# tky823/audio_source_separation

Hardware: AMD Instinct MI355X
Metric: ILRMA iterations/sec (4ch, F=1025, T=4096) (higher is better)
Workload: dtype f64; 1 GPU; gauss_ilrma_ip update_once, M=4 F=1025 T=4096 K=4, normalize=power, loss off; utterances_per_gpu=1, power_statistic=covariance, parallelism=utterance-sharded x1, no data-path collective

## Files before the change

audio_source_separation_amd/csrc/assx_bss.hip:

```cpp
#include "assx_common.hpp"
#include "assx_small_linalg.hpp"
#include "assx_stream.hpp"
#include "assx_group_linalg.hpp"
#include "assx_partition.hpp"
#include "assx_cov_wide.hpp"
#include "assx_cov_mfma.hpp"
#include "assx_nmf_internal.hpp"
#include "assx_widem.hpp"

using namespace assx;

namespace {

constexpr int REDUCE_THREADS = 256;

template <typename R, int M>
__device__ __forceinline__ void load_filter(const Cx<R>* __restrict__ W, size_t bf, Cx<R> (&w)[M][M]) {
  const Cx<R>* p = W + bf * (M * M);
#pragma unroll
  for (int n = 0; n < M; ++n)
#pragma unroll
    for (int m = 0; m < M; ++m) w[n][m] = p[n * M + m];
}

// ... 953 lines not shown
      hipLaunchKernelGGL((ip_par_kernel<R, M, false>), gp, bp, 0, st, (const Cx<R>*)U, (const R*)nullptr, fp, 1.0,
                         (Cx<R>*)W, (const Cx<R>*)C, pw, thr, status, B, F, den_floor, 1);
    ASSX_LAUNCH_CHECK(ctx, "ip_par_kernel");
    return 0;
  }
#endif
  const dim3 grid(blocks_for((size_t)B * F, GPW)), block(64);
  if (part)
    hipLaunchKernelGGL((ip_group_kernel<R, M, true>), grid, block, 0, st, (const Cx<R>*)nullptr, (const R*)part, fp,
                       1.0 / (double)T, (Cx<R>*)W, (const Cx<R>*)C, pw, thr, status, B, F, den_floor, wb);
  else
    hipLaunchKernelGGL((ip_group_kernel<R, M, false>), grid, block, 0, st, (const Cx<R>*)U, (const R*)nullptr, fp, 1.0,
                       (Cx<R>*)W, (const Cx<R>*)C, pw, thr, status, B, F, den_floor, 1);
  ASSX_LAUNCH_CHECK(ctx, "ip_group_kernel");
  return 0;
}

template <typename R, int M>
int run_iss(assx_ctx* ctx, const void* U, const void* part, FlatPart fp, int T, void* W, const void* C, double* pw,
            int B, int F, hipStream_t st) {
  constexpr int GPW = WAVE / next_pow2_c(M * M);
  const dim3 grid(blocks_for((size_t)B * F, GPW)), block(64);
  if (part)
    hipLaunchKernelGGL((iss_group_kernel<R, M, true>), grid, block, 0, st, (const Cx<R>*)nullptr, (const R*)part, fp,
                       1.0 / (double)T, (double)T, (Cx<R>*)W, (const Cx<R>*)C, pw, B, F);
  else
    hipLaunchKernelGGL((iss_group_kernel<R, M, false>), grid, block, 0, st, (const Cx<R>*)U, (const R*)nullptr, fp, 1.0,
                       (double)T, (Cx<R>*)W, (const Cx<R>*)C, pw, B, F);
  ASSX_LAUNCH_CHECK(ctx, "iss_group_kernel");
  return 0;
}

template <typename R, int M>
int run_ip2(assx_ctx* ctx, const void* U, const void* part, FlatPart fp, int T, void* W, const void* C, double* pw,
            double thr, int32_t* status, int B, int F, int pm, int pn, hipStream_t st) {
  constexpr int GPW = WAVE / next_pow2_c(M * M);
  const dim3 grid(blocks_for((size_t)B * F, GPW)), block(64);
  if (part)
    hipLaunchKernelGGL((ip2_group_kernel<R, M, true>), grid, block, 0, st, (const Cx<R>*)nullptr, (const R*)part, fp,
                       1.0 / (double)T, (Cx<R>*)W, (const Cx<R>*)C, pw, thr, status, B, F, pm, pn);
  else
    hipLaunchKernelGGL((ip2_group_kernel<R, M, false>), grid, block, 0, st, (const Cx<R>*)U, (const R*)nullptr, fp, 1.0,
                       (Cx<R>*)W, (const Cx<R>*)C, pw, thr, status, B, F, pm, pn);
  ASSX_LAUNCH_CHECK(ctx, "ip2_group_kernel");
  return 0;
}

template <typename R, int MM>
int run_basis_partial(assx_ctx* ctx, const void* X, const void* W, const void* Tb, const void* V, double domain,
                      double eps, void* ws, int B, int F, int T, int K, hipStream_t st, FlatPart* fp_out,
                      double nu = -1.0 ,
                      double* lpart = nullptr , int lstride = 0) {
  NmfArgs<R> a;
  a.nu = (R)nu;
  a.d = Dims{B, F, T, K};
  a.eps = (R)eps;
  a.p1 = make_pow((domain + 2.0) / domain);
  a.fp = flat_basis(B, F, T);
  *fp_out = a.fp;
  const bool d2 = a.p1.mode == POW_SQUARE, k4 = K <= KU;
  const dim3 gb(stream_grid(ctx, a.fp, B)), bb(64);
#define BASIS_LAUNCH(K4V, D2V, DXV, DWV, MW) \
  hipLaunchKernelGGL((basis_stream_kernel<R, MM, K4V, D2V, DXV, DWV, MW>), gb, bb, 0, st, (const Cx<R>*)X, \
                     (const Cx<R>*)W, (const R*)Tb, (const R*)V, (R*)ws, a)
  constexpr size_t vlds = (size_t)VDMA_SLOTS * VTileDma<R, MM * KU>::TILE_BYTES;
#define BASIS_VD(D2V, MW, TDV) \
  hipLaunchKernelGGL((basis_stream_vd_kernel<R, MM, D2V, 2, MW, TDV>), gb, bb, vlds, st, (const Cx<R>*)X, \
                     (const Cx<R>*)W, (const R*)Tb, (const R*)V, (R*)ws, a, (double*)nullptr, 0)
#if ASSX_LAB
  static const int vdma = lab_int("ASSX_BASIS_VDMA", 1);
  if (k4 && !vdma) {
    if (nu >= 0.0) hipLaunchKernelGGL((basis_stream_kernel<R, MM, true, true, 3, 1, 1, true>), gb, bb, 0, st, (const Cx<R>*)X,
                                      (const Cx<R>*)W, (const R*)Tb, (const R*)V, (R*)ws, a);
    else if (d2) BASIS_LAUNCH(true, true, 3, 1, 2);
    else BASIS_LAUNCH(true, false, 2, 1, 1);
  } else
#endif
  if (nu >= 0.0) {
    if (k4) BASIS_VD(true, 2, true);
    else hipLaunchKernelGGL((basis_stream_kernel<R, MM, false, true, 3, 1, 1, true>), gb, bb, 0, st, (const Cx<R>*)X,
                            (const Cx<R>*)W, (const R*)Tb, (const R*)V, (R*)ws, a);
  } else if (k4) {
    if (d2 && lpart)
      hipLaunchKernelGGL((basis_stream_vd_kernel<R, MM, true, 2, 2, false, true>), gb, bb, vlds, st, (const Cx<R>*)X,
                         (const Cx<R>*)W, (const R*)Tb, (const R*)V, (R*)ws, a, lpart, lstride);
    else if (d2) BASIS_VD(true, 2, false);
    else BASIS_VD(false, 1, false);
  } else if (d2) BASIS_LAUNCH(false, true, 3, 1, 1);
  else BASIS_LAUNCH(false, false, 2, 1, 1);
#undef BASIS_VD
#undef BASIS_LAUNCH
  ASSX_LAUNCH_CHECK(ctx, "basis_stream_kernel");
  return 0;
}

template <typename R, int MM>
int run_act_partial(assx_ctx* ctx, const void* X, const void* W, const void* Tb, const void* V, double domain,
                    double eps, void* ws, int B, int F, int T, int K, hipStream_t st, FlatPart* fp_out,
                    double nu = -1.0) {
  NmfArgs<R> a;
  a.nu = (R)nu;
  a.d = Dims{B, F, T, K};
  a.eps = (R)eps;
  a.p1 = make_pow((domain + 2.0) / domain);
  a.fp = flat_act(B, F, T);
  *fp_out = a.fp;
  const bool d2 = a.p1.mode == POW_SQUARE, k4 = K <= KU;
  const dim3 ga(stream_grid(ctx, a.fp, B)), ba(64 * ACT_NH);
#define ACT_LAUNCH(K4V, D2V, DXV, MW) \
  hipLaunchKernelGGL((act_stream_kernel<R, MM, K4V, D2V, DXV, MW>), ga, ba, 0, st, (const Cx<R>*)X, (const Cx<R>*)W, \
                     (const R*)Tb, (const R*)V, (R*)ws, a)
#define ACT_VD(D2V, DXV, MW, TDV) \
  hipLaunchKernelGGL((act_stream_vd_kernel<R, MM, D2V, DXV, MW, TDV>), ga, ba, 0, st, (const Cx<R>*)X, (const Cx<R>*)W, \
                     (const R*)Tb, (const R*)V, (R*)ws, a)
#if ASSX_LAB
  static const int vdma = lab_int("ASSX_ACT_VDMA", 1);
  if (k4 && !vdma) {
    if (nu >= 0.0) hipLaunchKernelGGL((act_stream_kernel<R, MM, true, true, 3, 1, true>), ga, ba, 0, st, (const Cx<R>*)X,
                                      (const Cx<R>*)W, (const R*)Tb, (const R*)V, (R*)ws, a);
    else if (d2) ACT_LAUNCH(true, true, (sizeof(R) == 8 ? 3 : 4), 2);
    else ACT_LAUNCH(true, false, 2, 1);
  } else
#endif
  if (nu >= 0.0) {
    if (k4) ACT_VD(true, 3, 2, true);
    else hipLaunchKernelGGL((act_stream_kernel<R, MM, false, true, 4, 1, true>), ga, ba, 0, st, (const Cx<R>*)X,
                            (const Cx<R>*)W, (const R*)Tb, (const R*)V, (R*)ws, a);
  } else if (k4) {
    if (d2) ACT_VD(true, 3, 2, false);
    else ACT_VD(false, 2, 1, false);
  } else if (d2) ACT_LAUNCH(false, true, 4, 1);
  else ACT_LAUNCH(false, false, 2, 1);
#undef ACT_VD
#undef ACT_LAUNCH
  ASSX_LAUNCH_CHECK(ctx, "act_stream_kernel");
  return 0;
}

template <typename R, int MM>
int run_cov_partial_tv(assx_ctx* ctx, const void* X, const void* Tb, const void* V, int K, double domain, double eps,
                       void* ws, void* U_dense, int B, int F, int T, int dtype, hipStream_t st, FlatPart* fp_out,
                       bool* dense, int* records_wb = nullptr ) {
  static const bool wide = lab_int("ASSX_WIDE_K", 1) != 0;
  static const bool fused = lab_int("ASSX_COV_WIDE", 1) != 0;
  *dense = false;
  if (records_wb) *records_wb = 1;
  if (K <= KU || !wide) return run_cov_partial<R, MM>(ctx, WK_TV, X, nullptr, Tb, V, K, domain, eps, ws, B, F, T, st, fp_out);
  const WsLayout L = ws_layout(B, MM, F, T, K, dtype);
  const PowSpec p2d = make_pow(2.0 / domain);
  static const bool mfma = lab_int("ASSX_COV_MFMA", 1) != 0;
  if (fused && mfma && U_dense && K <= 16 && (size_t)B * MM * K * T * sizeof(R) < 0xffffffffull) {
    const FlatPart fw = flat_cov_wide(B, F, T, 1);
    const Dims d{B, F, T, K};
    const int ks = (K + 3) / 4;
    const size_t ldsm = CovMfmaGeom<R>::lds_bytes(MM, ks);
    unsigned long long* covm_trace = COVM_TRACE ? (unsigned long long*)((char*)ws + L.total - 65536) : nullptr;
#define COVM_LAUNCH(D2V, KSV)                                                                                          \
  do {                                                                                                                 \
    if (ldsm > 64 * 1024) {                                                                                            \
      hipError_t e = hipFuncSetAttribute(reinterpret_cast<const void*>(cov_mfma_kernel<R, MM, D2V, KSV>),              \
                                         hipFuncAttributeMaxDynamicSharedMemorySize, (int)ldsm);                       \
      if (e != hipSuccess) return hip_fail(ctx, e, "hipFuncSetAttribute(cov_mfma_kernel)");                            \
    }                                                                                                                  \
    hipLaunchKernelGGL((cov_mfma_kernel<R, MM, D2V, KSV>), dim3(fw.G), dim3(WAVE * COVW_BINS), ldsm, st,               \
                       (const Cx<R>*)X, (const R*)Tb, (const R*)V, (R*)ws, d, fw, (R)eps, p2d, covm_trace);            \
  } while (0)
    if (p2d.mode == POW_ID) {
      if (ks == 2) COVM_LAUNCH(true, 2);
      else if (ks == 3) COVM_LAUNCH(true, 3);
      else COVM_LAUNCH(true, 4);
    } else {
      if (ks == 2) COVM_LAUNCH(false, 2);
      else if (ks == 3) COVM_LAUNCH(false, 3);
      else COVM_LAUNCH(false, 4);
    }
#undef COVM_LAUNCH
    ASSX_LAUNCH_CHECK(ctx, "cov_mfma_kernel");
    *fp_out = fw;
    if (records_wb) {
      *records_wb = COVW_BINS;
      return 0;
    }
    hipLaunchKernelGGL((cov_wide_finalize_kernel<R, MM>), dim3(blocks_for((size_t)B * MM * F * MM * MM, 256)), dim3(256),
                       0, st, (const R*)ws, (Cx<R>*)U_dense, B, F, fw, (R)(1.0 / (double)T));
    ASSX_LAUNCH_CHECK(ctx, "cov_wide_finalize_kernel");
    *dense = true;
    return 0;
  }
  const int sb = cov_wide_sb<R>(MM * K);
  const size_t lds = sb == 2 ? CovWideGeom<R, 2>::lds_bytes(MM * K) : CovWideGeom<R, 1>::lds_bytes(MM * K);
  if (fused && U_dense && lds <= 144 * 1024 && (size_t)B * MM * K * T * sizeof(R) < 0xffffffffull) {
    const FlatPart fw = flat_cov_wide(B, F, T, sb);
    const Dims d{B, F, T, K};
#define COVW_LAUNCH(D2V, SBV)                                                                                        \
  do {                                                                                                               \
    if (lds > 64 * 1024) {                                                                                           \
      hipError_t e = hipFuncSetAttribute(reinterpret_cast<const void*>(cov_wide_kernel<R, MM, D2V, SBV>),            \
                                         hipFuncAttributeMaxDynamicSharedMemorySize, (int)lds);                      \
      if (e != hipSuccess) return hip_fail(ctx, e, "hipFuncSetAttribute(cov_wide_kernel)");                          \
    }                                                                                                                \
    hipLaunchKernelGGL((cov_wide_kernel<R, MM, D2V, SBV>), dim3(fw.G), dim3(WAVE * COVW_BINS), lds, st,              \
                       (const Cx<R>*)X, (const R*)Tb, (const R*)V, (R*)ws, d, fw, (R)eps, p2d);                      \
  } while (0)
#if ASSX_LAB
    if (sb == 2) {
      if (p2d.mode == POW_ID) COVW_LAUNCH(true, 2);
      else COVW_LAUNCH(false, 2);
    } else
#endif
    if (p2d.mode == POW_ID) COVW_LAUNCH(true, 1);
    else COVW_LAUNCH(false, 1);
#undef COVW_LAUNCH
    ASSX_LAUNCH_CHECK(ctx, "cov_wide_kernel");
    if (records_wb) {
      *records_wb = COVW_BINS;
      *fp_out = fw;
      return 0;
    }
    hipLaunchKernelGGL((cov_wide_finalize_kernel<R, MM>), dim3(blocks_for((size_t)B * MM * F * MM * MM, 256)), dim3(256),
                       0, st, (const R*)ws, (Cx<R>*)U_dense, B, F, fw, (R)(1.0 / (double)T));
    ASSX_LAUNCH_CHECK(ctx, "cov_wide_finalize_kernel");
    *fp_out = fw;
    *dense = true;
    return 0;
  }
  R* rv = (R*)((char*)ws + L.map);
  const dim3 grid(blocks_for(T, 256), blocks_for(F, WIDE_FB), B * MM);
  if (p2d.mode == POW_ID)
    hipLaunchKernelGGL((source_variance_map_kernel<R, true>), grid, dim3(256), 0, st, (const R*)Tb, (const R*)V, rv, F, T,
                       K, p2d);
  else
    hipLaunchKernelGGL((source_variance_map_kernel<R, false>), grid, dim3(256), 0, st, (const R*)Tb, (const R*)V, rv, F,
                       T, K, p2d);
  ASSX_LAUNCH_CHECK(ctx, "source_variance_map_kernel");
  return run_cov_partial<R, MM>(ctx, WK_NFT, X, rv, nullptr, nullptr, 1, 2.0, eps, ws, B, F, T, st, fp_out);
}

}

extern "C" {

int assx_launch_order(int B, int F, int T, int reverse, int* ranges, int capacity) {
  if (B < 1 || F < 1 || T < 1) return ASSX_E_ARG;
  FlatPart fp = flat_cov(B, F, T, 1);
  const int grid = (int)set_launch_order(fp, B, reverse);
  if (ranges) {
    if (capacity < grid) return ASSX_E_ARG;
    for (int bid = 0; bid < grid; ++bid) ranges[bid] = workgroup_range(bid, grid, fp);
  }
  return grid;
}

size_t assx_workspace_bytes(int B, int M, int F, int T, int K, int dtype) {
  if (B < 1 || M < 1 || F < 1 || T < 1) return 0;
  if (widem::handles(M)) return widem::workspace_bytes(B, M, F, T, K, dtype);
  return ws_layout(B, M, F, T, K, dtype).total;
}

int assx_demix(assx_ctx* ctx, const void* X, const void* W, const void* scale, void* Y, int B, int M, int F, int T,
               int dtype, void* stream) {
  CHECK_COMMON(ctx, B, M, F, T);
  ASSX_REQUIRE(ctx, X && W && Y, ASSX_E_NULL, "assx_demix: NULL array");
  if (widem::handles(M)) return widem::demix(ctx, X, W, scale, Y, B, M, F, T, dtype, (hipStream_t)stream);
  hipStream_t st = (hipStream_t)stream;
  return dispatch_rm(ctx, dtype, M, [&](auto rt, auto mt) -> int {
    using R = decltype(rt);
    constexpr int MM = decltype(mt)::value;
    dim3 grid(blocks_for(T, 256), F, B);
    hipLaunchKernelGGL((demix_kernel<R, MM>), grid, dim3(256), 0, st, (const Cx<R>*)X, (const Cx<R>*)W,
                       (const Cx<R>*)scale, (Cx<R>*)Y, Dims{B, F, T, 0});
    ASSX_LAUNCH_CHECK(ctx, "demix_kernel");
    return 0;
  });
}

int assx_ilrma_power_map(assx_ctx* ctx, const void* X, const void* W, void* P, int B, int M, int F, int T, int dtype,
                         void* stream) {
  CHECK_COMMON(ctx, B, M, F, T);
  ASSX_REQUIRE(ctx, X && W && P, ASSX_E_NULL, "assx_ilrma_power_map: NULL array");
  hipStream_t st = (hipStream_t)stream;
  if (widem::handles(M)) return widem::power_map(ctx, X, W, P, B, M, F, T, dtype, st);
  return dispatch_rm(ctx, dtype, M, [&](auto rt, auto mt) -> int {
    using R = decltype(rt);
    constexpr int MM = decltype(mt)::value;
    hipLaunchKernelGGL((demix_power_map_kernel<R, MM>), dim3(blocks_for(T, 256), F, B), dim3(256), 0, st,
                       (const Cx<R>*)X, (const Cx<R>*)W, (R*)P, Dims{B, F, T, 0});
    ASSX_LAUNCH_CHECK(ctx, "demix_power_map_kernel");
    return 0;
  });
}

int assx_cov_accumulate(assx_ctx* ctx, const void* X, const void* r, int r_kind, double eps, void* U, void* ws, int B,
                        int M, int N, int F, int T, int dtype, void* stream) {
  CHECK_COMMON(ctx, B, M, F, T);
  ASSX_REQUIRE(ctx, X && U && ws, ASSX_E_NULL, "assx_cov_accumulate: NULL array");
  ASSX_REQUIRE(ctx, r_kind == ASSX_W_NONE || r_kind == ASSX_W_NT || r_kind == ASSX_W_NFT, ASSX_E_ARG,
               "assx_cov_accumulate: bad r_kind %d", r_kind);
  ASSX_REQUIRE(ctx, r_kind == ASSX_W_NONE ? (N == 1) : (N == M && r != nullptr), ASSX_E_ARG,
               "assx_cov_accumulate: N must be 1 (unweighted) or M with weights, got N=%d M=%d", N, M);
  if (widem::handles(M)) return widem::cov_accumulate(ctx, X, r, r_kind, eps, U, ws, B, M, N, F, T, dtype, (hipStream_t)stream);
  hipStream_t st = (hipStream_t)stream;
  return dispatch_rm(ctx, dtype, M, [&](auto rt, auto mt) -> int {
    using R = decltype(rt);
    constexpr int MM = decltype(mt)::value;
    return run_cov<R, MM>(ctx, r_kind, X, r, nullptr, nullptr, 1, 2.0, eps, U, ws, B, F, T, st);
  });
}

int assx_ip_update(assx_ctx* ctx, const void* U, void* W, double threshold, int32_t* status, int B, int M, int F,
                   int dtype, void* stream) {
  CHECK_COMMON(ctx, B, M, F, 1);
  ASSX_REQUIRE(ctx, U && W, ASSX_E_NULL, "assx_ip_update: NULL array");
  if (widem::handles(M)) return widem::ip_update(ctx, U, W, threshold, status, B, M, F, dtype, (hipStream_t)stream);
  hipStream_t st = (hipStream_t)stream;
  return dispatch_rm(ctx, dtype, M, [&](auto rt, auto mt) -> int {
    using R = decltype(rt);
    constexpr int MM = decltype(mt)::value;
    return run_ip<R, MM>(ctx, U, nullptr, FlatPart{}, 1, W, nullptr, nullptr, threshold, status, B, F, st);
  });
}

int assx_ip2_update(assx_ctx* ctx, const void* U, void* W, double threshold, int32_t* status, int pair_m, int pair_n,
                    int B, int M, int F, int dtype, void* stream) {
  CHECK_COMMON(ctx, B, M, F, 1);
  ASSX_REQUIRE(ctx, U && W, ASSX_E_NULL, "assx_ip2_update: NULL array");
  ASSX_REQUIRE(ctx, pair_m >= 0 && pair_m < M && pair_n >= 0 && pair_n < M && pair_m != pair_n, ASSX_E_ARG,
               "bad update pair (%d, %d) for %d sources", pair_m, pair_n, M);
// ... 831 lines not shown
```

audio_source_separation_amd/csrc/assx_cov_mfma.hpp:

```cpp
#pragma once
#include "assx_cov_wide.hpp"
#include "assx_nmf_mfma.hpp"

#ifndef COVM_TRACE
#define COVM_TRACE 0
#endif
#ifndef COVM_SKIP
#define COVM_SKIP 0
#endif

#if (COVM_SKIP || COVM_TRACE) && !defined(ASSX_PROBE_BUILD)
#error "COVM_SKIP / COVM_TRACE are timing experiments (wrong results by construction): build them with -DASSX_PROBE_BUILD into a probe library, never into libassx.so"
#endif

namespace assx {

template <typename R>
struct CovMfmaRows;
template <>
struct CovMfmaRows<double> {
  static __device__ __forceinline__ int bin_of_row(int i) { return i < COVW_BINS ? i : -1; }
  static __device__ __forceinline__ int bin_of_reg(int lane, int r) { return (lane >> 4) + 4 * r; }
};
template <>
struct CovMfmaRows<float> {
  static __device__ __forceinline__ int bin_of_row(int i) { return (i & 3) < 2 ? 2 * (i >> 2) + (i & 3) : -1; }
  static __device__ __forceinline__ int bin_of_reg(int lane, int r) { return 2 * (lane >> 4) + r; }
};

template <int M>
__host__ __device__ constexpr int herm_pair_m(int p) {
  int m = 0;
  while (p >= M - 1 - m) {
    p -= M - 1 - m;
    ++m;
  }
  return m;
}
template <int M>
__host__ __device__ constexpr int herm_pair_l(int p) {
  int m = 0;
  while (p >= M - 1 - m) {
    p -= M - 1 - m;
    ++m;
  }
  return m + 1 + p;
}

template <typename R>
struct CovMfmaGeom {
  static constexpr int DXS = 3;
  static constexpr int RB = WAVE * 2 * (int)sizeof(R);
  static constexpr int LPR = RB / 16;
  static constexpr int RPI = WAVE / LPR;
  static __host__ __device__ constexpr int nxi(int M) { return (M + RPI - 1) / RPI; }
  static __host__ __device__ constexpr int mp(int M) { return nxi(M) * RPI; }
  static __host__ __device__ constexpr size_t x_bytes(int M) { return (size_t)DXS * COVW_BINS * mp(M) * RB; }
  static __host__ __device__ constexpr size_t lds_bytes(int M, int KS) {
    return x_bytes(M) + ((size_t)2 * M * COVW_BINS * WAVE + (size_t)2 * M * 16 * 4 * KS) * sizeof(R);
  }
};

template <int RB>
__device__ __forceinline__ void xrows_read(unsigned addr, Vec2<double> (&x)[4]) {
  asm volatile("ds_read_b128 %0, %4\n\tds_read_b128 %1, %4 offset:%5\n\tds_read_b128 %2, %4 offset:%6\n\t"
               "ds_read_b128 %3, %4 offset:%7"
               : "=&v"(x[0]), "=&v"(x[1]), "=&v"(x[2]), "=&v"(x[3])
               : "v"(addr), "n"(RB), "n"(2 * RB), "n"(3 * RB)
               : "memory");
}
template <int RB>
__device__ __forceinline__ void xrows_read(unsigned addr, Vec2<double> (&x)[3]) {
  asm volatile("ds_read_b128 %0, %3\n\tds_read_b128 %1, %3 offset:%4\n\tds_read_b128 %2, %3 offset:%5"
               : "=&v"(x[0]), "=&v"(x[1]), "=&v"(x[2])
               : "v"(addr), "n"(RB), "n"(2 * RB)
               : "memory");
}
template <int RB>
__device__ __forceinline__ void xrows_read(unsigned addr, Vec2<double> (&x)[2]) {
  asm volatile("ds_read_b128 %0, %2\n\tds_read_b128 %1, %2 offset:%3"
               : "=&v"(x[0]), "=&v"(x[1])
               : "v"(addr), "n"(RB)
               : "memory");
}
template <int RB>
__device__ __forceinline__ void xrows_read(unsigned addr, Vec2<float> (&x)[4]) {
  asm volatile("ds_read_b64 %0, %4\n\tds_read_b64 %1, %4 offset:%5\n\tds_read_b64 %2, %4 offset:%6\n\t"
               "ds_read_b64 %3, %4 offset:%7"
               : "=&v"(x[0]), "=&v"(x[1]), "=&v"(x[2]), "=&v"(x[3])
               : "v"(addr), "n"(RB), "n"(2 * RB), "n"(3 * RB)
               : "memory");
}
template <int RB>
__device__ __forceinline__ void xrows_read(unsigned addr, Vec2<float> (&x)[3]) {
  asm volatile("ds_read_b64 %0, %3\n\tds_read_b64 %1, %3 offset:%4\n\tds_read_b64 %2, %3 offset:%5"
               : "=&v"(x[0]), "=&v"(x[1]), "=&v"(x[2])
               : "v"(addr), "n"(RB), "n"(2 * RB)
               : "memory");
}
template <int RB>
__device__ __forceinline__ void xrows_read(unsigned addr, Vec2<float> (&x)[2]) {
  asm volatile("ds_read_b64 %0, %2\n\tds_read_b64 %1, %2 offset:%3"
               : "=&v"(x[0]), "=&v"(x[1])
               : "v"(addr), "n"(RB)
               : "memory");
}

template <typename R, int M>
__device__ __forceinline__ void xrows_wait(Vec2<R> (&x)[M]) {
  asm volatile("s_waitcnt lgkmcnt(0)" ::: "memory");
#pragma unroll
  for (int m = 0; m < M; ++m) asm volatile("" : "+v"(x[m]));
}

template <int N, typename R, int NV>
__device__ __forceinline__ void wait_values(R (&v)[NV]) {
  asm volatile("s_waitcnt vmcnt(%0)" ::"n"(N) : "memory");
#pragma unroll
  for (int i = 0; i < NV; ++i) asm volatile("" : "+v"(v[i]));
}

template <typename R, int M, bool D2, int KS>
__global__ void __launch_bounds__(WAVE * COVW_BINS)
    cov_mfma_kernel(const Cx<R>* __restrict__ X, const R* __restrict__ Tb, const R* __restrict__ V, R* __restrict__ part,
                    Dims d, FlatPart fp, R eps, PowSpec p2d, unsigned long long* trace) {
#if defined(__HIP_DEVICE_COMPILE__)
  constexpr int N = M, HM = M * M, WB = COVW_BINS, NACC = N * HM, NV = next_pow2_c(NACC);
  constexpr int KP = 4 * KS;
  constexpr int NT = (4 * N + WB - 1) / WB;
  constexpr int NB = NT * KS;
  using MM = Mfma16<R>;
  using acc_t = typename MM::acc_t;
  using ROWS = CovMfmaRows<R>;
  using GEO = CovMfmaGeom<R>;
  constexpr int NXI = GEO::nxi(M), MP = GEO::mp(M), RB = GEO::RB, DXS = GEO::DXS;
  int trace_n = 0;
  auto stamp = [&]() {
    if (COVM_TRACE && trace && blockIdx.x == 100 && (threadIdx.x == 0 || threadIdx.x == 320) && trace_n < 400)
      trace[(threadIdx.x ? 400 : 0) + trace_n] = __builtin_amdgcn_s_memtime();
    ++trace_n;
  };
  const int F = d.F, T = d.T, K = d.K, TBk = fp.len, FG = (F + WB - 1) / WB;
  extern __shared__ __attribute__((aligned(16))) unsigned char smem[];
  R* const Wt = reinterpret_cast<R*>(smem + GEO::x_bytes(M));
  R* const Tl = Wt + 2 * N * WB * WAVE;
  const int tid = threadIdx.x, lane = tid & (WAVE - 1);
  const int w = __builtin_amdgcn_readfirstlane(tid >> 6);
  const int li = lane & 15, lk = lane >> 4;
  const int g = (int)blockIdx.x;
  long long q0, q1;
  flat_range(fp, g, q0, q1);
  if (q0 >= q1) return;
  const int nblk = (int)(q1 - q0);
  const int jg_first = (int)(q0 / TBk);
  Cursor c0;
  c0.tb = (int)(q0 - (long long)jg_first * TBk);
  c0.b = jg_first / FG;
  c0.f = jg_first - c0.b * FG;
  const size_t FT = (size_t)F * T;
  unsigned char* const xring = smem + (size_t)w * MP * RB;
  const unsigned xread0 = (unsigned)(size_t)(__attribute__((address_space(3))) void*)xring + (unsigned)lane * (unsigned)sizeof(Cx<R>);
  constexpr unsigned SLOT_BYTES = (unsigned)WB * MP * RB;

  const int jt = w & 3;
  auto tile_src = [&](int i) { return (w >> 2) + 2 * i; };
  auto tile_on = [&](int i) { return (4 * N) % WB == 0 || w + WB * i < 4 * N; };

  auto load_rows = [&](const Cursor& c, int par) {
    for (int i = tid; i < N * 16 * KP; i += WAVE * WB) {
      const int n = i / (16 * KP), rem = i - n * 16 * KP, row = rem / KP, k = rem - row * KP;
      const int bin = ROWS::bin_of_row(row), ff = c.f * WB + bin;
      R v = 0;
      if (bin >= 0 && ff < F && k < K) v = Tb[(((size_t)c.b * N + n) * F + ff) * K + k];
      Tl[par * (N * 16 * KP) + i] = v;
    }
  };
  const unsigned xlane = (unsigned)((size_t)(lane / GEO::LPR) * FT * sizeof(Cx<R>)) + (unsigned)(lane % GEO::LPR) * 16u;
  const unsigned xlast = (unsigned)((size_t)(min((NXI - 1) * GEO::RPI + lane / GEO::LPR, M - 1) - (NXI - 1) * GEO::RPI) * FT * sizeof(Cx<R>)) +
                         (unsigned)(lane % GEO::LPR) * 16u;
  struct XReq {
    BufRsrc rx;
    unsigned row;
    unsigned char* slot;
  };
  auto x_item = [&](const Cursor& c, int sl) {
    XReq q;
    q.rx = make_rsrc_sized(X + (size_t)c.b * M * FT, (size_t)M * FT * sizeof(Cx<R>));
    q.row = (unsigned)(((size_t)min(c.f * WB + w, F - 1) * T + (size_t)c.tb * WAVE) * sizeof(Cx<R>));
    q.slot = xring + (unsigned)sl * SLOT_BYTES;
    return q;
  };
  auto request_x1 = [&](const XReq& q, auto jc) {
    constexpr int j = decltype(jc)::value;
    const unsigned voff = (j == NXI - 1 ? xlast : xlane) + (q.row + (unsigned)((size_t)j * GEO::RPI * FT * sizeof(Cx<R>)));
    __builtin_amdgcn_raw_ptr_buffer_load_lds(q.rx, (__attribute__((address_space(3))) void*)(q.slot + j * GEO::RPI * RB), 16,
                                             (int)voff, 0, 0, 0);
  };
  unsigned vlane[NT], vlastl[NT];
#pragma unroll
  for (int i = 0; i < NT; ++i) {
    const int n = min(tile_src(i), N - 1);
    vlane[i] = (unsigned)(((size_t)(n * K + lk) * T + 16 * jt + li) * sizeof(R));
    vlastl[i] = (unsigned)(((size_t)(n * K + min(4 * (KS - 1) + lk, K - 1)) * T + 16 * jt + li) * sizeof(R));
  }
  struct VReq {
    buf_u4 rv;
    unsigned col;
  };
  auto v_item = [&](const Cursor& c) {
    VReq q;
    q.rv = make_rsrc_words(V + (size_t)c.b * N * K * T, (size_t)N * K * T * sizeof(R));
    q.rv.x = __builtin_amdgcn_readfirstlane(q.rv.x);
    q.rv.y = __builtin_amdgcn_readfirstlane(q.rv.y);
    q.rv.z = __builtin_amdgcn_readfirstlane(q.rv.z);
    q.rv.w = __builtin_amdgcn_readfirstlane(q.rv.w);
    q.col = (unsigned)__builtin_amdgcn_readfirstlane((int)((size_t)c.tb * WAVE * sizeof(R)));
    return q;
  };
  auto request_v1 = [&](const VReq& q, R (&bv)[NB], auto ic, auto sc) {
    constexpr int i = decltype(ic)::value, s2 = decltype(sc)::value;
    const unsigned voff = (s2 == KS - 1 ? vlastl[i] : vlane[i] + (unsigned)((size_t)4 * s2 * T * sizeof(R))) + q.col;
    buf_ld_tied(bv[i * KS + s2], q.rv, voff, 0u);
  };
  auto request_v = [&](const Cursor& c, R (&bv)[NB]) {
    const VReq q = v_item(c);
    static_for<NT>([&](auto ic) { static_for<KS>([&](auto sc) { request_v1(q, bv, ic, sc); }); });
  };
  auto request_x = [&](const Cursor& c, int sl) {
    const XReq q = x_item(c, sl);
    static_for<NXI>([&](auto jc) { request_x1(q, jc); });
  };
  auto read_rows = [&](int par, R (&av)[NT][KS]) {
#pragma unroll
    for (int i = 0; i < NT; ++i)
#pragma unroll
      for (int s2 = 0; s2 < KS; ++s2) av[i][s2] = Tl[((par * N + min(tile_src(i), N - 1)) * 16 + li) * KP + 4 * s2 + lk];
  };
  auto variance = [&](int par, const R (&bv)[NB], acc_t (&tv)[NT]) {
    R av[NT][KS];
    read_rows(par, av);
#pragma unroll
    for (int i = 0; i < NT; ++i)
#pragma unroll
      for (int r = 0; r < 4; ++r) tv[i][r] = 0;
#pragma unroll
    for (int s2 = 0; s2 < KS; ++s2)
#pragma unroll
      for (int i = 0; i < NT; ++i)
        if (tile_on(i)) tv[i] = MM::mma(av[i][s2], bv[i * KS + s2], tv[i]);
  };
  auto publish = [&](const Cursor& c, int buf, const acc_t (&tv)[NT], auto&& between) {
    constexpr int NC = 2 * NT;
    const bool tlive = c.tb * WAVE + 16 * jt + li < T;
    R rr[NC], rc[NC], er[NC];
#pragma unroll
    for (int q = 0; q < NC; ++q)
      rr[q] = floor_eps<R>(D2 ? tv[q / 2][q % 2] : powspec<R>(tv[q / 2][q % 2], p2d), eps);
    between(IntC<0>());
#pragma unroll
    for (int q = 0; q < NC; ++q) rc[q] = sizeof(R) == 8 ? (R)__builtin_amdgcn_rcp((double)rr[q]) : (R)__builtin_amdgcn_rcpf((float)rr[q]);
    between(IntC<1>());
#pragma unroll
    for (int q = 0; q < NC; ++q) er[q] = fma(-rr[q], rc[q], (R)1);
#pragma unroll
    for (int q = 0; q < NC; ++q) rc[q] = fma(rc[q], er[q], rc[q]);
    between(IntC<2>());
    if (sizeof(R) == 8) {
#pragma unroll
      for (int q = 0; q < NC; ++q) er[q] = fma(-rr[q], rc[q], (R)1);
#pragma unroll
      for (int q = 0; q < NC; ++q) rc[q] = fma(rc[q], er[q], rc[q]);
    }
    between(IntC<3>());
#pragma unroll
    for (int q = 0; q < NC; ++q) asm volatile("" : "+v"(rc[q]));
#pragma unroll
    for (int q = 0; q < NC; ++q) {
      const int i = q / 2, bin = ROWS::bin_of_reg(lane, q % 2);
      if (tile_on(i)) Wt[((buf * N + tile_src(i)) * WB + bin) * WAVE + 16 * jt + li] = (tlive && c.f * WB + bin < F) ? rc[q] : (R)0;
    }
  };
  auto nothing = [](auto) {};

  R acc[NV];
#pragma unroll
  for (int q = 0; q < NV; ++q) acc[q] = 0;
  R bn[NB];
#pragma unroll
  for (int i = 0; i < NB; ++i) bn[i] = 0;
  acc_t tv[NT], tvp[NT];
  Cursor c1 = c0;
  advance(c1, TBk, FG);
  Cursor c2 = c1;
  advance(c2, TBk, FG);
  Cursor c3 = c2;
  advance(c3, TBk, FG);
  int par = 0;
  load_rows(c0, 0);
  request_v(c0, bn);
  request_x(c0, 0);
  wait_values<0>(bn);
  __syncthreads();
  variance(0, bn, tv);
  publish(c0, 0, tv, nothing);
  {
    const Cursor c1v = nblk > 1 ? c1 : c0, c2v = nblk > 2 ? c2 : c0;
    if (nblk > 1 && c1.tb == 0) {
      par = 1;
      load_rows(c1, 1);
      __syncthreads();
    }
    request_v(c1v, bn);
    wait_values<0>(bn);
    variance(par, bn, tvp);
    if (nblk > 2 && c2.tb == 0) {
      par ^= 1;
      load_rows(c2, par);
    }
    request_v(c2v, bn);
    request_x(c1v, 1);
  }
  int sl = 0;
  for (int it = 0; it < nblk; ++it) {
    const bool more = it + 1 < nblk, more2 = it + 2 < nblk, more3 = it + 3 < nblk;
    stamp();
    wait_values<(COVM_SKIP & 4) ? 0 : NXI>(bn);
    stamp();
    Vec2<R> xv[M];
    xrows_read<RB>(xread0 + (unsigned)sl * SLOT_BYTES, xv);
    if (!(COVM_SKIP & 16)) asm volatile("s_waitcnt lgkmcnt(0)\n\ts_barrier" ::: "memory");
    stamp();
    Cursor c1v = c1, c2v = c2, c3v = c3;
    if (!more) c1v = c0;
    if (!more2) c2v = c0;
    if (!more3) c3v = c0;
    const int sl2 = sl == 0 ? DXS - 1 : sl - 1;
    R wgt[N];
#pragma unroll
    for (int n = 0; n < N; ++n) wgt[n] = Wt[(((it & 1) * N + n) * WB + w) * WAVE + lane];
    R av[NT][KS];
    read_rows(par, av);
    const VReq vq = v_item(c3v);
    const XReq xq = x_item(c2v, sl2);
    __builtin_amdgcn_sched_barrier(0);
    if (!(COVM_SKIP & 8)) publish(c1v, (it + 1) & 1, tvp, [&](auto) { __builtin_amdgcn_sched_barrier(0); });
    __builtin_amdgcn_sched_barrier(0);
    stamp();
    xrows_wait(xv);
    Cx<R> x[M];
#pragma unroll
    for (int m = 0; m < M; ++m) x[m] = cmake<R>(xv[m].x, xv[m].y);
#pragma unroll
    for (int i = 0; i < NT; ++i)
#pragma unroll
      for (int r = 0; r < 4; ++r) tv[i][r] = 0;
    constexpr int NU = M + M * (M - 1) / 2;
    auto fan_unit = [&](auto uc) {
      constexpr int u = decltype(uc)::value;
      if constexpr (u < M) {
        const R pd = cabs2(x[u]);
#pragma unroll
        for (int n = 0; n < N; ++n) acc[n * HM + u] = fma(wgt[n], pd, acc[n * HM + u]);
      } else {
        constexpr int m = herm_pair_m<M>(u - M), l = herm_pair_l<M>(u - M);
        const Cx<R> pr = cmulc(x[m], x[l]);
        constexpr int hb = herm_pair_base<M>(m, l);
#pragma unroll
        for (int n = 0; n < N; ++n) {
          acc[n * HM + hb] = fma(wgt[n], pr.x, acc[n * HM + hb]);
          acc[n * HM + hb + 1] = fma(wgt[n], pr.y, acc[n * HM + hb + 1]);
        }
      }
    };
    constexpr int NSTEP = NB + NXI;
    static_for<NSTEP>([&](auto qc) {
      constexpr int q = decltype(qc)::value;
      if constexpr (q < NB) {
        constexpr int sq = q / NT, iq = q % NT;
        if (!(COVM_SKIP & 1))
          if (tile_on(iq)) tv[iq] = MM::mma(av[iq][sq], bn[iq * KS + sq], tv[iq]);
        if (!(COVM_SKIP & 32)) request_v1(vq, bn, IntC<iq>(), IntC<sq>());
      } else {
        if (!(COVM_SKIP & 4)) request_x1(xq, IntC<q - NB>());
      }
      __builtin_amdgcn_sched_barrier(0);
      if (!(COVM_SKIP & 2)) static_for<(q + 1) * NU / NSTEP - q * NU / NSTEP>([&](auto jc) { fan_unit(IntC<q * NU / NSTEP + decltype(jc)::value>()); });
      __builtin_amdgcn_sched_barrier(0);
    });
    value_fence(acc);
    stamp();
#pragma unroll
    for (int i = 0; i < NT; ++i) tvp[i] = tv[i];
    if (more3 && c3.tb == 0) load_rows(c3, par ^ 1);
    if (c1.tb == 0 || !more) {
      const R tot = wave_reduce_scatter<R, NV>(acc);
      const int i = scatter_index<NV>();
      const int slot = c0.b * FG + c0.f - jg_first;
      if (scatter_leader<NV>() && i < NACC) part[(((size_t)g * fp.S + slot) * WB + w) * NACC + i] = tot;
#pragma unroll
      for (int q = 0; q < NV; ++q) acc[q] = 0;
    }
    if (more3 && c3.tb == 0) par ^= 1;
    sl = sl + 1 == DXS ? 0 : sl + 1;
    c0 = c1;
    c1 = c2;
    c2 = c3;
    advance(c3, TBk, FG);
    stamp();
  }
  asm volatile("s_waitcnt vmcnt(0)" ::: "memory");
#endif
}

}
```

Before: 5585 iterations/s.

## Pack two sources per MFMA variance tile and pad LDS weight stride

```diff
diff --git a/audio_source_separation_amd/csrc/assx_bss.hip b/audio_source_separation_amd/csrc/assx_bss.hip
--- a/audio_source_separation_amd/csrc/assx_bss.hip
+++ b/audio_source_separation_amd/csrc/assx_bss.hip
@@ -1129,8 +1129,8 @@
   if (fused && mfma && U_dense && K <= 16 && (size_t)B * MM * K * T * sizeof(R) < 0xffffffffull) {
     const FlatPart fw = flat_cov_wide(B, F, T, 1);
     const Dims d{B, F, T, K};
-    const int ks = (K + 3) / 4;
-    const size_t ldsm = CovMfmaGeom<R>::lds_bytes(MM, ks);
+    const int ks = (2 * K + 3) / 4, kse = (ks + 1) & ~1;
+    const size_t ldsm = CovMfmaGeom<R>::lds_bytes(MM, p2d.mode == POW_ID ? ks : kse);
     unsigned long long* covm_trace = COVM_TRACE ? (unsigned long long*)((char*)ws + L.total - 65536) : nullptr;
 #define COVM_LAUNCH(D2V, KSV)                                                                                          \
   do {                                                                                                                 \
@@ -1143,13 +1143,16 @@
                        (const Cx<R>*)X, (const R*)Tb, (const R*)V, (R*)ws, d, fw, (R)eps, p2d, covm_trace);            \
   } while (0)
     if (p2d.mode == POW_ID) {
-      if (ks == 2) COVM_LAUNCH(true, 2);
-      else if (ks == 3) COVM_LAUNCH(true, 3);
-      else COVM_LAUNCH(true, 4);
+      if (ks == 3) COVM_LAUNCH(true, 3);
+      else if (ks == 4) COVM_LAUNCH(true, 4);
+      else if (ks == 5) COVM_LAUNCH(true, 5);
+      else if (ks == 6) COVM_LAUNCH(true, 6);
+      else if (ks == 7) COVM_LAUNCH(true, 7);
+      else COVM_LAUNCH(true, 8);
     } else {
-      if (ks == 2) COVM_LAUNCH(false, 2);
-      else if (ks == 3) COVM_LAUNCH(false, 3);
-      else COVM_LAUNCH(false, 4);
+      if (kse == 4) COVM_LAUNCH(false, 4);
+      else if (kse == 6) COVM_LAUNCH(false, 6);
+      else COVM_LAUNCH(false, 8);
     }
 #undef COVM_LAUNCH
     ASSX_LAUNCH_CHECK(ctx, "cov_mfma_kernel");
diff --git a/audio_source_separation_amd/csrc/assx_cov_mfma.hpp b/audio_source_separation_amd/csrc/assx_cov_mfma.hpp
--- a/audio_source_separation_amd/csrc/assx_cov_mfma.hpp
+++ b/audio_source_separation_amd/csrc/assx_cov_mfma.hpp
@@ -9,6 +9,10 @@
 #define COVM_SKIP 0
 #endif
 
+#ifndef COVM_WPAD
+#define COVM_WPAD 1
+#endif
+
 #if (COVM_SKIP || COVM_TRACE) && !defined(ASSX_PROBE_BUILD)
 #error "COVM_SKIP / COVM_TRACE are timing experiments (wrong results by construction): build them with -DASSX_PROBE_BUILD into a probe library, never into libassx.so"
 #endif
@@ -19,12 +23,14 @@
 struct CovMfmaRows;
 template <>
 struct CovMfmaRows<double> {
-  static __device__ __forceinline__ int bin_of_row(int i) { return i < COVW_BINS ? i : -1; }
+  static __device__ __forceinline__ int src_of_row(int i) { return i >> 3; }
+  static __device__ __forceinline__ int bin_of_row(int i) { return i & 7; }
   static __device__ __forceinline__ int bin_of_reg(int lane, int r) { return (lane >> 4) + 4 * r; }
 };
 template <>
 struct CovMfmaRows<float> {
-  static __device__ __forceinline__ int bin_of_row(int i) { return (i & 3) < 2 ? 2 * (i >> 2) + (i & 3) : -1; }
+  static __device__ __forceinline__ int src_of_row(int i) { return (i & 3) >> 1; }
+  static __device__ __forceinline__ int bin_of_row(int i) { return 2 * (i >> 2) + (i & 1); }
   static __device__ __forceinline__ int bin_of_reg(int lane, int r) { return 2 * (lane >> 4) + r; }
 };
 
@@ -56,8 +62,11 @@
   static __host__ __device__ constexpr int nxi(int M) { return (M + RPI - 1) / RPI; }
   static __host__ __device__ constexpr int mp(int M) { return nxi(M) * RPI; }
   static __host__ __device__ constexpr size_t x_bytes(int M) { return (size_t)DXS * COVW_BINS * mp(M) * RB; }
+  static constexpr int WSTR = COVM_WPAD ? WAVE + (sizeof(R) == 8 ? 16 : 8) : WAVE;
+  static __host__ __device__ constexpr int row_ld(int KS) { return 4 * KS + (sizeof(R) == 8 ? 1 : 2); }
+  static __host__ __device__ constexpr int pairs(int M) { return (M + 1) / 2; }
   static __host__ __device__ constexpr size_t lds_bytes(int M, int KS) {
-    return x_bytes(M) + ((size_t)2 * M * COVW_BINS * WAVE + (size_t)2 * M * 16 * 4 * KS) * sizeof(R);
+    return x_bytes(M) + ((size_t)2 * M * COVW_BINS * WSTR + (size_t)2 * pairs(M) * 16 * row_ld(KS)) * sizeof(R);
   }
 };
 
@@ -127,13 +136,14 @@
 #if defined(__HIP_DEVICE_COMPILE__)
   constexpr int N = M, HM = M * M, WB = COVW_BINS, NACC = N * HM, NV = next_pow2_c(NACC);
   constexpr int KP = 4 * KS;
-  constexpr int NT = (4 * N + WB - 1) / WB;
-  constexpr int NB = NT * KS;
+  constexpr int NP = (N + 1) / 2;
+  constexpr int NB = KS;
+  static_assert(4 * NP <= WB, "one variance tile per wave");
   using MM = Mfma16<R>;
   using acc_t = typename MM::acc_t;
   using ROWS = CovMfmaRows<R>;
   using GEO = CovMfmaGeom<R>;
-  constexpr int NXI = GEO::nxi(M), MP = GEO::mp(M), RB = GEO::RB, DXS = GEO::DXS;
+  constexpr int NXI = GEO::nxi(M), MP = GEO::mp(M), RB = GEO::RB, DXS = GEO::DXS, WSTR = GEO::WSTR, LD = GEO::row_ld(KS);
   int trace_n = 0;
   auto stamp = [&]() {
     if (COVM_TRACE && trace && blockIdx.x == 100 && (threadIdx.x == 0 || threadIdx.x == 320) && trace_n < 400)
@@ -143,7 +153,7 @@
   const int F = d.F, T = d.T, K = d.K, TBk = fp.len, FG = (F + WB - 1) / WB;
   extern __shared__ __attribute__((aligned(16))) unsigned char smem[];
   R* const Wt = reinterpret_cast<R*>(smem + GEO::x_bytes(M));
-  R* const Tl = Wt + 2 * N * WB * WAVE;
+  R* const Tl = Wt + 2 * N * WB * WSTR;
   const int tid = threadIdx.x, lane = tid & (WAVE - 1);
   const int w = __builtin_amdgcn_readfirstlane(tid >> 6);
   const int li = lane & 15, lk = lane >> 4;
@@ -151,41 +161,41 @@
   long long q0, q1;
   flat_range(fp, g, q0, q1);
   if (q0 >= q1) return;
-  const int nblk = (int)(q1 - q0);
-  const int jg_first = (int)(q0 / TBk);
+  const int nblk = __builtin_amdgcn_readfirstlane((int)(q1 - q0));
+  const int jg_first = __builtin_amdgcn_readfirstlane((int)(q0 / TBk));
   Cursor c0;
-  c0.tb = (int)(q0 - (long long)jg_first * TBk);
-  c0.b = jg_first / FG;
-  c0.f = jg_first - c0.b * FG;
+  c0.tb = __builtin_amdgcn_readfirstlane((int)(q0 - (long long)jg_first * TBk));
+  c0.b = __builtin_amdgcn_readfirstlane(jg_first / FG);
+  c0.f = __builtin_amdgcn_readfirstlane(jg_first - c0.b * FG);
+  const int b0 = c0.b;
   const size_t FT = (size_t)F * T;
   unsigned char* const xring = smem + (size_t)w * MP * RB;
   const unsigned xread0 = (unsigned)(size_t)(__attribute__((address_space(3))) void*)xring + (unsigned)lane * (unsigned)sizeof(Cx<R>);
   constexpr unsigned SLOT_BYTES = (unsigned)WB * MP * RB;
 
   const int jt = w & 3;
-  auto tile_src = [&](int i) { return (w >> 2) + 2 * i; };
-  auto tile_on = [&](int i) { return (4 * N) % WB == 0 || w + WB * i < 4 * N; };
+  const bool tile_on = 4 * NP == WB || w < 4 * NP;
+  const int tp = tile_on ? w >> 2 : 0;
 
   auto load_rows = [&](const Cursor& c, int par) {
-    for (int i = tid; i < N * 16 * KP; i += WAVE * WB) {
-      const int n = i / (16 * KP), rem = i - n * 16 * KP, row = rem / KP, k = rem - row * KP;
-      const int bin = ROWS::bin_of_row(row), ff = c.f * WB + bin;
+    for (int i = tid; i < NP * 16 * KP; i += WAVE * WB) {
+      const int pp = i / (16 * KP), rem = i - pp * 16 * KP, row = rem / KP, cc = rem - row * KP;
+      const int s = ROWS::src_of_row(row), n = 2 * pp + s, k = cc - s * K, ff = c.f * WB + ROWS::bin_of_row(row);
       R v = 0;
-      if (bin >= 0 && ff < F && k < K) v = Tb[(((size_t)c.b * N + n) * F + ff) * K + k];
-      Tl[par * (N * 16 * KP) + i] = v;
+      if (n < N && ff < F && k >= 0 && k < K) v = Tb[(((size_t)b0 * N + n) * F + ff) * K + k];
+      Tl[((par * NP + pp) * 16 + row) * LD + cc] = v;
     }
   };
   const unsigned xlane = (unsigned)((size_t)(lane / GEO::LPR) * FT * sizeof(Cx<R>)) + (unsigned)(lane % GEO::LPR) * 16u;
   const unsigned xlast = (unsigned)((size_t)(min((NXI - 1) * GEO::RPI + lane / GEO::LPR, M - 1) - (NXI - 1) * GEO::RPI) * FT * sizeof(Cx<R>)) +
                          (unsigned)(lane % GEO::LPR) * 16u;
+  const BufRsrc rx = make_rsrc_sized(X + (size_t)b0 * M * FT, (size_t)M * FT * sizeof(Cx<R>));
   struct XReq {
-    BufRsrc rx;
     unsigned row;
     unsigned char* slot;
   };
   auto x_item = [&](const Cursor& c, int sl) {
     XReq q;
-    q.rx = make_rsrc_sized(X + (size_t)c.b * M * FT, (size_t)M * FT * sizeof(Cx<R>));
     q.row = (unsigned)(((size_t)min(c.f * WB + w, F - 1) * T + (size_t)c.tb * WAVE) * sizeof(Cx<R>));
     q.slot = xring + (unsigned)sl * SLOT_BYTES;
     return q;
@@ -193,69 +203,65 @@
   auto request_x1 = [&](const XReq& q, auto jc) {
     constexpr int j = decltype(jc)::value;
     const unsigned voff = (j == NXI - 1 ? xlast : xlane) + (q.row + (unsigned)((size_t)j * GEO::RPI * FT * sizeof(Cx<R>)));
-    __builtin_amdgcn_raw_ptr_buffer_load_lds(q.rx, (__attribute__((address_space(3))) void*)(q.slot + j * GEO::RPI * RB), 16,
+    __builtin_amdgcn_raw_ptr_buffer_load_lds(rx, (__attribute__((address_space(3))) void*)(q.slot + j * GEO::RPI * RB), 16,
                                              (int)voff, 0, 0, 0);
   };
-  unsigned vlane[NT], vlastl[NT];
-#pragma unroll
-  for (int i = 0; i < NT; ++i) {
-    const int n = min(tile_src(i), N - 1);
-    vlane[i] = (unsigned)(((size_t)(n * K + lk) * T + 16 * jt + li) * sizeof(R));
-    vlastl[i] = (unsigned)(((size_t)(n * K + min(4 * (KS - 1) + lk, K - 1)) * T + 16 * jt + li) * sizeof(R));
-  }
+  unsigned vrow[KS];
+#pragma unroll
+  for (int s2 = 0; s2 < KS; ++s2) {
+    const int cc = min(4 * s2 + lk, 2 * K - 1), sr = cc >= K ? 1 : 0, n = min(2 * tp + sr, N - 1);
+    vrow[s2] = (unsigned)(((size_t)(n * K + cc - sr * K) * T + 16 * jt + li) * sizeof(R));
+  }
+  buf_u4 rv = make_rsrc_words(V + (size_t)b0 * N * K * T, (size_t)N * K * T * sizeof(R));
+  rv.x = __builtin_amdgcn_readfirstlane(rv.x);
+  rv.y = __builtin_amdgcn_readfirstlane(rv.y);
+  rv.z = __builtin_amdgcn_readfirstlane(rv.z);
+  rv.w = __builtin_amdgcn_readfirstlane(rv.w);
   struct VReq {
-    buf_u4 rv;
     unsigned col;
   };
   auto v_item = [&](const Cursor& c) {
     VReq q;
-    q.rv = make_rsrc_words(V + (size_t)c.b * N * K * T, (size_t)N * K * T * sizeof(R));
-    q.rv.x = __builtin_amdgcn_readfirstlane(q.rv.x);
-    q.rv.y = __builtin_amdgcn_readfirstlane(q.rv.y);
-    q.rv.z = __builtin_amdgcn_readfirstlane(q.rv.z);
-    q.rv.w = __builtin_amdgcn_readfirstlane(q.rv.w);
     q.col = (unsigned)__builtin_amdgcn_readfirstlane((int)((size_t)c.tb * WAVE * sizeof(R)));
     return q;
   };
-  auto request_v1 = [&](const VReq& q, R (&bv)[NB], auto ic, auto sc) {
-    constexpr int i = decltype(ic)::value, s2 = decltype(sc)::value;
-    const unsigned voff = (s2 == KS - 1 ? vlastl[i] : vlane[i] + (unsigned)((size_t)4 * s2 * T * sizeof(R))) + q.col;
-    buf_ld_tied(bv[i * KS + s2], q.rv, voff, 0u);
+  auto request_v1 = [&](const VReq& q, R (&bv)[NB], auto sc) {
+    constexpr int s2 = decltype(sc)::value;
+    buf_ld_tied(bv[s2], rv, vrow[s2] + q.col, 0u);
   };
   auto request_v = [&](const Cursor& c, R (&bv)[NB]) {
     const VReq q = v_item(c);
-    static_for<NT>([&](auto ic) { static_for<KS>([&](auto sc) { request_v1(q, bv, ic, sc); }); });
+    static_for<KS>([&](auto sc) { request_v1(q, bv, sc); });
   };
   auto request_x = [&](const Cursor& c, int sl) {
     const XReq q = x_item(c, sl);
     static_for<NXI>([&](auto jc) { request_x1(q, jc); });
   };
-  auto read_rows = [&](int par, R (&av)[NT][KS]) {
-#pragma unroll
-    for (int i = 0; i < NT; ++i)
-#pragma unroll
-      for (int s2 = 0; s2 < KS; ++s2) av[i][s2] = Tl[((par * N + min(tile_src(i), N - 1)) * 16 + li) * KP + 4 * s2 + lk];
-  };
-  auto variance = [&](int par, const R (&bv)[NB], acc_t (&tv)[NT]) {
-    R av[NT][KS];
+  auto read_rows = [&](int par, R (&av)[KS]) {
+#pragma unroll
+    for (int s2 = 0; s2 < KS; ++s2) av[s2] = Tl[((par * NP + tp) * 16 + li) * LD + 4 * s2 + lk];
+  };
+  auto product = [&](R a, R b, acc_t& tv, auto sc) {
+    if constexpr (decltype(sc)::value == 0) {
+      const acc_t zero = {0, 0, 0, 0};
+      tv = MM::mma(a, b, zero);
+    } else {
+      tv = MM::mma(a, b, tv);
+    }
+  };
+  auto variance = [&](int par, const R (&bv)[NB], acc_t& tv) {
+    R av[KS];
     read_rows(par, av);
-#pragma unroll
-    for (int i = 0; i < NT; ++i)
-#pragma unroll
-      for (int r = 0; r < 4; ++r) tv[i][r] = 0;
-#pragma unroll
-    for (int s2 = 0; s2 < KS; ++s2)
-#pragma unroll
-      for (int i = 0; i < NT; ++i)
-        if (tile_on(i)) tv[i] = MM::mma(av[i][s2], bv[i * KS + s2], tv[i]);
-  };
-  auto publish = [&](const Cursor& c, int buf, const acc_t (&tv)[NT], auto&& between) {
-    constexpr int NC = 2 * NT;
+    if (tile_on) static_for<KS>([&](auto sc) { product(av[decltype(sc)::value], bv[decltype(sc)::value], tv, sc); });
+  };
+  const int wlane[2] = {ROWS::bin_of_reg(lane, 0) * WSTR + 16 * jt + li, ROWS::bin_of_reg(lane, 1) * WSTR + 16 * jt + li};
+  auto publish = [&](const Cursor& c, int buf, const acc_t& tv, auto&& between) {
+    constexpr int NC = 4;
     const bool tlive = c.tb * WAVE + 16 * jt + li < T;
     R rr[NC], rc[NC], er[NC];
 #pragma unroll
     for (int q = 0; q < NC; ++q)
-      rr[q] = floor_eps<R>(D2 ? tv[q / 2][q % 2] : powspec<R>(tv[q / 2][q % 2], p2d), eps);
+      rr[q] = floor_eps<R>(D2 ? tv[q] : powspec<R>(tv[q], p2d), eps);
     between(IntC<0>());
 #pragma unroll
     for (int q = 0; q < NC; ++q) rc[q] = sizeof(R) == 8 ? (R)__builtin_amdgcn_rcp((double)rr[q]) : (R)__builtin_amdgcn_rcpf((float)rr[q]);
@@ -276,8 +282,8 @@
     for (int q = 0; q < NC; ++q) asm volatile("" : "+v"(rc[q]));
 #pragma unroll
     for (int q = 0; q < NC; ++q) {
-      const int i = q / 2, bin = ROWS::bin_of_reg(lane, q % 2);
-      if (tile_on(i)) Wt[((buf * N + tile_src(i)) * WB + bin) * WAVE + 16 * jt + li] = (tlive && c.f * WB + bin < F) ? rc[q] : (R)0;
+      const int n = 2 * tp + q / 2, bin = ROWS::bin_of_reg(lane, q % 2);
+      if (tile_on && n < N) Wt[(buf * N + n) * (WB * WSTR) + wlane[q % 2]] = (tlive && c.f * WB + bin < F) ? rc[q] : (R)0;
     }
   };
   auto nothing = [](auto) {};
@@ -288,7 +294,7 @@
   R bn[NB];
 #pragma unroll
   for (int i = 0; i < NB; ++i) bn[i] = 0;
-  acc_t tv[NT], tvp[NT];
+  acc_t tv = {0, 0, 0, 0};
   Cursor c1 = c0;
   advance(c1, TBk, FG);
   Cursor c2 = c1;
@@ -312,7 +318,7 @@
     }
     request_v(c1v, bn);
     wait_values<0>(bn);
-    variance(par, bn, tvp);
+    variance(par, bn, tv);
     if (nblk > 2 && c2.tb == 0) {
       par ^= 1;
       load_rows(c2, par);
@@ -337,23 +343,19 @@
     const int sl2 = sl == 0 ? DXS - 1 : sl - 1;
     R wgt[N];
 #pragma unroll
-    for (int n = 0; n < N; ++n) wgt[n] = Wt[(((it & 1) * N + n) * WB + w) * WAVE + lane];
-    R av[NT][KS];
+    for (int n = 0; n < N; ++n) wgt[n] = Wt[(((it & 1) * N + n) * WB + w) * WSTR + lane];
+    R av[KS];
     read_rows(par, av);
     const VReq vq = v_item(c3v);
     const XReq xq = x_item(c2v, sl2);
     __builtin_amdgcn_sched_barrier(0);
-    if (!(COVM_SKIP & 8)) publish(c1v, (it + 1) & 1, tvp, [&](auto) { __builtin_amdgcn_sched_barrier(0); });
+    if (!(COVM_SKIP & 8)) publish(c1v, (it + 1) & 1, tv, [&](auto) { __builtin_amdgcn_sched_barrier(0); });
     __builtin_amdgcn_sched_barrier(0);
     stamp();
     xrows_wait(xv);
     Cx<R> x[M];
 #pragma unroll
     for (int m = 0; m < M; ++m) x[m] = cmake<R>(xv[m].x, xv[m].y);
-#pragma unroll
-    for (int i = 0; i < NT; ++i)
-#pragma unroll
-      for (int r = 0; r < 4; ++r) tv[i][r] = 0;
     constexpr int NU = M + M * (M - 1) / 2;
     auto fan_unit = [&](auto uc) {
       constexpr int u = decltype(uc)::value;
@@ -376,10 +378,9 @@
     static_for<NSTEP>([&](auto qc) {
       constexpr int q = decltype(qc)::value;
       if constexpr (q < NB) {
-        constexpr int sq = q / NT, iq = q % NT;
         if (!(COVM_SKIP & 1))
-          if (tile_on(iq)) tv[iq] = MM::mma(av[iq][sq], bn[iq * KS + sq], tv[iq]);
-        if (!(COVM_SKIP & 32)) request_v1(vq, bn, IntC<iq>(), IntC<sq>());
+          if (tile_on) product(av[q], bn[q], tv, qc);
+        if (!(COVM_SKIP & 32)) request_v1(vq, bn, qc);
       } else {
         if (!(COVM_SKIP & 4)) request_x1(xq, IntC<q - NB>());
       }
@@ -389,8 +390,6 @@
     });
     value_fence(acc);
     stamp();
-#pragma unroll
-    for (int i = 0; i < NT; ++i) tvp[i] = tv[i];
     if (more3 && c3.tb == 0) load_rows(c3, par ^ 1);
     if (c1.tb == 0 || !more) {
       const R tot = wave_reduce_scatter<R, NV>(acc);
```

After: 5567 iterations/s. About the same (-0.3%).
